# ndrwmlnk/critic-guided-segmentation-of-rewarding-objects-in-first-person-views

Hardware: AMD Instinct MI355X
Metric: Hourglass+critic train images/sec, 64x64x3 batch=512 (higher is better)
Workload: dtype f32

## Files before the change

critic-guided-segmentation-of-rewarding-objects-in-first-person-views_amd/csrc/mask_head.hip:

```cpp
#include "wgrad_body.h"

struct MHeadParams {
    const float* dzpre; const float* h; const float* w2; const float* w0;
    const void* img;
    const float* o0;
    float* dh;
    float* d_o0;
    float* slab2;
    float* slab0;
    int n, ntiles;
    unsigned long long* dbg;
};

#ifdef CGS_DEBUG_STAMPS
#define MH_T() __builtin_amdgcn_s_memtime()
static unsigned long long* g_mh_stamps = nullptr;
extern "C" int dbg_mask_head_stamps(unsigned long long* stamps) { g_mh_stamps = stamps; return CGS_OK; }
#else
#define MH_T() 0ull
#endif

#ifndef MH_WACC_PK
#define MH_WACC_PK 1
#endif
#ifndef MH_APK
#define MH_APK 1
#endif
#ifndef MH_INTERLEAVE
#define MH_INTERLEAVE 1
#endif
#ifndef MH_DGRAD4
#define MH_DGRAD4 1
#endif
#ifndef MH_DZWIN
#define MH_DZWIN 1
#endif
template <int TH, bool W0>
struct MHeadGeo {
    static constexpr int H = 64, W = 64, TRA = TH + 2, PW = W + 2, PS = 17, DZW = W + 4, DZR = TH + 4, STRIPS = H / TH;
    static constexpr int XT = TRA * PW * PS, DZ = DZR * DZW;
    static constexpr int W4P = MH_DGRAD4 ? 16 * 16 * 8 : 24 * 16 * 16;
    static constexpr int LR = TH / 2 + 2, LC = W / 2 + 2;
    static constexpr int XIMG = W0 ? TRA * PW * 4 : 0, XO = W0 ? LR * LC * 8 : 0;
    static constexpr int FLOATS = 2 * XT + 2 * XIMG + 2 * XO + W4P + 2 * DZ;
    static constexpr size_t LDS = (size_t)((FLOATS + 3) / 4) * 16;
    static constexpr int RED2 = 0, REDA = 1024, REDB = REDA + 4 * 32 * 16, RED_END = REDB + 4 * 4 * 32 * 16;
    static_assert(RED_END <= 2 * XT, "reduction buffers fit in the tile storage");
};

struct MHeadLds { float *xt0, *ximg, *xo, *w4p, *dz; };

template <int TH, bool WG, bool W0, int SRC>
__device__ __forceinline__ void mask_head_builder(const MHeadParams& P, const MHeadLds& L, const int btid, const int T,
                                                  const int bid, const int grid) {
    using G = MHeadGeo<TH, W0>;
    constexpr int H = G::H, W = G::W, TRA = G::TRA, PW = G::PW, PS = G::PS, DZW = G::DZW, LR = G::LR, LC = G::LC;
    constexpr int IT = TRA * W * 4 / 256, DIT = (G::DZ + 255) / 256;
    constexpr int NPIX = TRA * PW, NLO = LR * LC * 2, ITA = (NPIX + 255) / 256, ITB = (NLO + 255) / 256;
    static_assert((TRA * W * 4) % 256 == 0, "whole iterations: no element is visited twice");
    const int lane = btid & 63, wave = btid >> 6;
    const int pl = btid & 3;
    static_assert(4 * W == 256, "one tile row per 256-thread item");
    const int bx = btid >> 2, bx4 = btid;
    auto tile_of = [&](int i) { return bid + (i < T ? i : T - 1) * grid; };

    float w2r[9][4];
#if MH_APK
    typedef float mh_f2 __attribute__((ext_vector_type(2)));
    mh_f2 w2p[9][2];
#endif
#if MH_WACC_PK
#if !MH_APK
    typedef float mh_f2 __attribute__((ext_vector_type(2)));
#endif
    mh_f2 wacc[9][2];
#else
    float wacc[9][4];
#endif
    float bacc = 0.f;
    float4 hvs[IT];
    float dzr[DIT];
#pragma unroll
    for (int t = 0; t < 9; ++t)
#pragma unroll
        for (int c = 0; c < 4; ++c) {
            w2r[t][c] = P.w2[t * 16 + 4 * pl + c];
#if MH_APK
            w2p[t][c >> 1][c & 1] = w2r[t][c];
#endif
#if MH_WACC_PK
            wacc[t][c >> 1][c & 1] = 0.f;
#else
            wacc[t][c] = 0.f;
#endif
        }

    auto load_h_into = [&](float4 (&dst)[IT], int tile) {
        const int n0 = tile / G::STRIPS, row0 = (tile % G::STRIPS) * TH;
#pragma unroll
        for (int it = 0; it < IT; ++it) {
            const int y = row0 + it - 1;
            const bool in = y >= 0 && y < H;
            dst[it] = ((const float4*)P.h)[(in ? (n0 * H + y) * W * 4 : 0) + bx4];
        }
    };
    auto load_h = [&](int tile) { load_h_into(hvs, tile); };
    auto load_dz = [&](int tile) {
        const int n0 = tile / G::STRIPS, row0 = (tile % G::STRIPS) * TH;
#pragma unroll
        for (int it = 0; it < DIT; ++it) {
            int e = btid + it * 256;
            e = e < G::DZ ? e : G::DZ - 1;
            int y = row0 + e / DZW - 2, x = e % DZW - 2;
            bool in = y >= 0 && y < H && x >= 0 && x < W;
            dzr[it] = P.dzpre[in ? (n0 * H + y) * W + x : 0];
        }
    };
    auto store_dz = [&](int tile, int buf) {
        const int row0 = (tile % G::STRIPS) * TH;
        float* const dzb = L.dz + buf * G::DZ;
#pragma unroll
        for (int it = 0; it < DIT; ++it) {
            int e = btid + it * 256;
            e = e < G::DZ ? e : G::DZ - 1;
            int y = row0 + e / DZW - 2, x = e % DZW - 2;
            bool in = y >= 0 && y < H && x >= 0 && x < W;
            dzb[e] = in ? dzr[it] : 0.f;
        }
    };

    [[maybe_unused]] float4 ra[W0 ? ITA : 1], rb[W0 ? ITB : 1];
    auto fetch_x = [&](int tile) {
        const int n0 = tile / G::STRIPS, row0 = (tile % G::STRIPS) * TH;
#pragma unroll
        for (int it = 0; it < ITA; ++it) {
            int e = btid + it * 256; e = e < NPIX ? e : NPIX - 1;
            int y = row0 + e / PW - 1, x = e % PW - 1;
            bool in = y >= 0 && y < H && x >= 0 && x < W;
            int pix = in ? (n0 * H + y) * W + x : 0;
            if constexpr (SRC == WSRC_U8) {
                const uint32_t* s32 = (const uint32_t*)P.img;
                int off = pix * 3, last = P.n * H * W * 3 / 4 - 1, d = off >> 2;
                ra[it].x = __uint_as_float(s32[d]);
                ra[it].y = __uint_as_float(s32[d + 1 <= last ? d + 1 : last]);
            } else {
                const float* sf = (const float*)P.img;
                ra[it] = make_float4(sf[pix * 3], sf[pix * 3 + 1], sf[pix * 3 + 2], 0.f);
            }
        }
#pragma unroll
        for (int it = 0; it < ITB; ++it) {
            int e = btid + it * 256; e = e < NLO ? e : NLO - 1;
            int half = e & 1, pc = (e >> 1) % LC, pr = (e >> 1) / LC;
            int ly = row0 / 2 + pr - 1, lx = pc - 1;
            bool in = ly >= 0 && ly < H / 2 && lx >= 0 && lx < W / 2;
            rb[it] = ((const float4*)P.o0)[in ? ((n0 * (H / 2) + ly) * (W / 2) + lx) * 2 + half : 0];
        }
    };
    auto commit_x = [&](int tile, int buf) {
        const int n0 = tile / G::STRIPS, row0 = (tile % G::STRIPS) * TH;
        float4* const ximg4 = (float4*)(L.ximg + buf * G::XIMG);
        float4* const xo4 = (float4*)(L.xo + buf * G::XO);
#pragma unroll
        for (int it = 0; it < ITA; ++it) {
            int e = btid + it * 256; e = e < NPIX ? e : NPIX - 1;
            int y = row0 + e / PW - 1, x = e % PW - 1;
            bool in = y >= 0 && y < H && x >= 0 && x < W;
            float4 v = ra[it];
            if constexpr (SRC == WSRC_U8) {
                int pix = in ? (n0 * H + y) * W + x : 0;
                const uint32_t lo = __float_as_uint(v.x), hi = __float_as_uint(v.y);
                const uint32_t b3 = __builtin_amdgcn_alignbyte(hi, lo, (uint32_t)((pix * 3) & 3));
                const float sc = 1.f / 255.f;
                v = make_float4((float)(b3 & 255u) * sc, (float)((b3 >> 8) & 255u) * sc, (float)((b3 >> 16) & 255u) * sc, 0.f);
            }
            v.w = 0.f;
            ximg4[e] = in ? v : f4zero();
        }
#pragma unroll
        for (int it = 0; it < ITB; ++it) {
            int e = btid + it * 256; e = e < NLO ? e : NLO - 1;
            int pc = (e >> 1) % LC, pr = (e >> 1) / LC;
            int ly = row0 / 2 + pr - 1, lx = pc - 1;
            bool in = ly >= 0 && ly < H / 2 && lx >= 0 && lx < W / 2;
            xo4[e] = in ? rb[it] : f4zero();
        }
    };
    load_dz(tile_of(0));
    load_h(tile_of(0));
    store_dz(tile_of(0), 0);
    __syncthreads();

    [[maybe_unused]] unsigned long long tp = MH_T(), s_p1 = 0, s_w1 = 0, s_p2 = 0, s_w2 = 0;
    for (int i = 0; i <= T; ++i) {
        [[maybe_unused]] const unsigned long long tb = MH_T();
        [[maybe_unused]] unsigned long long tc = tb;
        if (i < T) {
            const int tile = tile_of(i);
            const int n0 = tile / G::STRIPS, row0 = (tile % G::STRIPS) * TH;
            float* xt = L.xt0 + (i & 1) * G::XT;
            const float* dz = L.dz + (i & 1) * G::DZ;
            load_dz(tile_of(i + 1));
            if constexpr (W0) fetch_x(tile);
            __builtin_amdgcn_sched_barrier(0);
#ifdef MH_WHATIF_NOBUILD
            if (P.n < 0)
#endif
            {
#if MH_DZWIN
            float dzw[IT + 2][3];
#pragma unroll
            for (int rr = 0; rr < IT + 2; ++rr)
#pragma unroll
                for (int cc = 0; cc < 3; ++cc) dzw[rr][cc] = dz[rr * DZW + bx + 1 + cc];
            __builtin_amdgcn_sched_barrier(0);
#endif
#pragma unroll
            for (int it = 0; it < IT; ++it) {
                const int r = it;
                const int x = bx, y = row0 + it - 1;
                const bool in = (it >= 1 && it <= TH) || (y >= 0 && y < H);
                const int gi = (in ? (n0 * H + y) * W * 4 : 0) + bx4;
                const float4 hv = hvs[it];
                const bool own = it >= 1 && it <= TH;
                const float4 hw_ = own ? hv : f4zero();
#if MH_APK
                mh_f2 a01 = {0.f, 0.f}, a23 = {0.f, 0.f};
#else
                float a0 = 0.f, a1 = 0.f, a2 = 0.f, a3 = 0.f;
#endif
#pragma unroll
                for (int ky = 0; ky < 3; ++ky)
#pragma unroll
                    for (int kx = 0; kx < 3; ++kx) {
#if MH_DZWIN
                        float d = dzw[r + 2 - ky][2 - kx];
#else
                        float d = dz[(r + 2 - ky) * DZW + x + 3 - kx];
#endif
#if MH_APK
                        {
                            const mh_f2 dd = {d, d};
                            a01 = __builtin_elementwise_fma(dd, w2p[ky * 3 + kx][0], a01);
                            a23 = __builtin_elementwise_fma(dd, w2p[ky * 3 + kx][1], a23);
                        }
#else
                        a0 = fmaf(d, w2r[ky * 3 + kx][0], a0); a1 = fmaf(d, w2r[ky * 3 + kx][1], a1);
                        a2 = fmaf(d, w2r[ky * 3 + kx][2], a2); a3 = fmaf(d, w2r[ky * 3 + kx][3], a3);
#endif
                        if (WG && it != 0 && it != IT - 1) {
#if MH_WACC_PK
                            const mh_f2 dd = {d, d};
                            wacc[ky * 3 + kx][0] = __builtin_elementwise_fma(dd, mh_f2{hw_.x, hw_.y}, wacc[ky * 3 + kx][0]);
                            wacc[ky * 3 + kx][1] = __builtin_elementwise_fma(dd, mh_f2{hw_.z, hw_.w}, wacc[ky * 3 + kx][1]);
#else
                            wacc[ky * 3 + kx][0] = fmaf(d, hw_.x, wacc[ky * 3 + kx][0]);
                            wacc[ky * 3 + kx][1] = fmaf(d, hw_.y, wacc[ky * 3 + kx][1]);
                            wacc[ky * 3 + kx][2] = fmaf(d, hw_.z, wacc[ky * 3 + kx][2]);
                            wacc[ky * 3 + kx][3] = fmaf(d, hw_.w, wacc[ky * 3 + kx][3]);
#endif
                        }
                    }
#if MH_APK
                const float a0 = a01[0], a1 = a01[1], a2 = a23[0], a3 = a23[1];
#endif
                static_assert(IT == TH + 2, "one item per tile row: item index == row index");
                if (WG && it != 0 && it != IT - 1) {
#if MH_DZWIN
                    bacc += (own && pl == 0) ? dzw[r + 1][1] : 0.f;
#else
                    bacc += (own && pl == 0) ? dz[(r + 1) * DZW + x + 2] : 0.f;
#endif
#pragma unroll
                    for (int t = 0; t < 9; ++t)
#pragma unroll
#if MH_WACC_PK
                        for (int c = 0; c < 2; ++c) asm volatile("" : "+v"(wacc[t][c]));
#else
                        for (int c = 0; c < 4; ++c) asm volatile("" : "+v"(wacc[t][c]));
#endif
                }
                float4 v = make_float4(a0 * (hv.x > 0.f ? 1.f : 0.01f), a1 * (hv.y > 0.f ? 1.f : 0.01f),
                                       a2 * (hv.z > 0.f ? 1.f : 0.01f), a3 * (hv.w > 0.f ? 1.f : 0.01f));
                v = in ? v : f4zero();
                float* d = xt + (r * PW + x + 1) * PS + 4 * pl;
                d[0] = v.x; d[1] = v.y; d[2] = v.z; d[3] = v.w;
                if (own && P.dh) ((float4*)P.dh)[gi] = v;
                __builtin_amdgcn_sched_barrier(0);
            }
            }
            load_h(tile_of(i + 1));
            tc = MH_T();
            store_dz(tile_of(i + 1), (i + 1) & 1);
            if constexpr (W0) commit_x(tile, i & 1);
        }
        [[maybe_unused]] const unsigned long long te = MH_T();
        __syncthreads();
        if (CGS_STAMP_PTR(P.dbg)) { const unsigned long long td = MH_T(); s_p1 += te - tc; s_p2 += tc - tb; s_w2 += td - te; tp = td; }
    }
    if (CGS_STAMP_PTR(P.dbg) && btid == 0) {
        unsigned long long* o = CGS_STAMP_PTR(P.dbg) + (size_t)bid * 16;
        o[0] = s_p1; o[1] = s_w1; o[2] = s_p2; o[3] = s_w2; o[4] = (unsigned long long)T;
    }

    if constexpr (WG) {
        float* red2 = L.xt0 + G::RED2;
#pragma unroll
        for (int t = 0; t < 9; ++t)
#pragma unroll
            for (int c = 0; c < 4; ++c) {
#if MH_WACC_PK
                float v = wacc[t][c >> 1][c & 1];
#else
                float v = wacc[t][c];
#endif
                v += __shfl_xor(v, 4, 64); v += __shfl_xor(v, 8, 64); v += __shfl_xor(v, 16, 64); v += __shfl_xor(v, 32, 64);
                if (lane < 4) red2[(wave * 4 + lane) * 37 + t * 4 + c] = v;
            }
        float v = bacc;
        v += __shfl_xor(v, 4, 64); v += __shfl_xor(v, 8, 64); v += __shfl_xor(v, 16, 64); v += __shfl_xor(v, 32, 64);
        if (lane < 4) red2[(wave * 4 + lane) * 37 + 36] = v;
    }
}

template <int TH, bool W0, int SRC>
__device__ __forceinline__ void mask_head_matrix(const MHeadParams& P, const MHeadLds& L, const int mtid, const int T,
                                                 const int bid, const int grid) {
    using G = MHeadGeo<TH, W0>;
    constexpr int PW = G::PW, PS = G::PS, LC = G::LC;
    static_assert(TH == 8, "4 matrix waves: one low-res row (data gradient) and one even + one odd row (weight gradient) each");
    const int lane = mtid & 63, mwave = mtid >> 6;
    const int l15 = lane & 15, kq = lane >> 4;
    auto tile_of = [&](int i) { return bid + (i < T ? i : T - 1) * grid; };
    frag4 accA[2], accB[2][2][2];
#pragma unroll
    for (int q = 0; q < 2; ++q) {
        accA[q] = frag4{0.f, 0.f, 0.f, 0.f};
#pragma unroll
        for (int c = 0; c < 4; ++c) accB[c >> 1][c & 1][q] = frag4{0.f, 0.f, 0.f, 0.f};
    }
    int rimg[2];
#pragma unroll
    for (int q = 0; q < 2; ++q) {
        int r = 16 * q + l15, tap = r / 3, c = r % 3;
        rimg[q] = r < 27 ? ((tap / 3) * PW + tap % 3) * 4 + c : 0;
    }
    const float m1 = (16 + l15 < 27) ? 1.f : 0.f, m0 = (16 + l15 == 27) ? 1.f : 0.f;

    [[maybe_unused]] float w4r[2][16];
    if constexpr (MH_DGRAD4) {
        if (mwave < 2) {
#pragma unroll
            for (int g = 0; g < 2; ++g)
#pragma unroll
                for (int k = 0; k < 16; ++k) w4r[g][k] = L.w4p[(k * 16 + (lane >> 2)) * 8 + 4 * g + (lane & 3)];
        }
    }
    [[maybe_unused]] unsigned long long tp = MH_T(), s_p1 = 0, s_w1 = 0, s_dg = 0, s_wg = 0, s_w2 = 0, tm = 0;
    __syncthreads();
    for (int i = 0; i <= T; ++i) {
        [[maybe_unused]] const unsigned long long ta = MH_T();
        [[maybe_unused]] const unsigned long long tb = ta;
        if (i > 0) {
            const int tile = tile_of(i - 1);
            const int n0 = tile / G::STRIPS, row0 = (tile % G::STRIPS) * TH;
            const float* xt = L.xt0 + ((i - 1) & 1) * G::XT;
            [[maybe_unused]] const float* const ximg = L.ximg + ((i - 1) & 1) * G::XIMG;
            [[maybe_unused]] const float* const xo = L.xo + ((i - 1) & 1) * G::XO;
#ifdef MH_WHATIF_NODGRAD
            if (P.n < 0)
#endif
            if constexpr (MH_DGRAD4) {
                if (mwave < 2) {
                    const int qyl = 2 * mwave + (lane >> 5), qx = lane & 31;
                    const float* bp = xt + ((2 * qyl) * PW + 2 * qx) * PS;
                    frag4 d0 = frag4{0.f, 0.f, 0.f, 0.f}, d1 = frag4{0.f, 0.f, 0.f, 0.f};
                    float bv[2][16];
                    auto ldp = [&](int k, int buf) {
#pragma unroll
                        for (int oc = 0; oc < 16; ++oc) bv[buf][oc] = bp[((k >> 2) * PW + (k & 3)) * PS + oc];
                    };
                    ldp(0, 0);
                    static_for<16>([&](auto K) {
                        constexpr int k = decltype(K)::value;
                        if constexpr (k + 1 < 16) ldp(k + 1, (k + 1) & 1);
                        __builtin_amdgcn_sched_barrier(0);
                        static_for<16>([&](auto OC) {
                            constexpr int oc = decltype(OC)::value;
                            d0 = __builtin_amdgcn_mfma_f32_4x4x1f32(w4r[0][k], bv[k & 1][oc], d0, 4, oc, 0);
                            d1 = __builtin_amdgcn_mfma_f32_4x4x1f32(w4r[1][k], bv[k & 1][oc], d1, 4, oc, 0);
                        });
                        __builtin_amdgcn_sched_barrier(0);
                    });
                    float4* o = (float4*)(P.d_o0 + ((size_t)(n0 * 32 + row0 / 2 + qyl) * 32 + qx) * 8);
                    o[0] = make_float4(d0[0], d0[1], d0[2], d0[3]);
                    o[1] = make_float4(d1[0], d1[1], d1[2], d1[3]);
                }
            } else {
                const int qyl = mwave;
                const int abase = ((2 * qyl) * PW + 4 * l15) * PS + kq;
                const float* wb = L.w4p + kq * 16 + l15;
                frag4 d = frag4{0.f, 0.f, 0.f, 0.f}, d1 = frag4{0.f, 0.f, 0.f, 0.f};
                constexpr int GS = 12, NG = 96 / GS;
                float av[2][GS], bw[2][GS];
                auto ld = [&](int g, int buf) {
#pragma unroll
                    for (int j = 0; j < GS; ++j) {
                        const int s = g * GS + j, pos = s >> 2, u = pos / 6, v6 = pos % 6;
                        av[buf][j] = xt[abase + (u * PW + v6) * PS + 4 * (s & 3)];
                        bw[buf][j] = wb[s * 64];
                    }
                };
                ld(0, 0);
                __builtin_amdgcn_sched_barrier(0);
#pragma unroll
                for (int g = 0; g < NG; ++g) {
                    if (g + 1 < NG) ld(g + 1, (g + 1) & 1);
#if !MH_INTERLEAVE
                    __builtin_amdgcn_sched_barrier(0);
#endif
#pragma unroll
                    for (int j = 0; j < GS; j += 2) {
                        d = __builtin_amdgcn_mfma_f32_16x16x4f32(av[g & 1][j], bw[g & 1][j], d, 0, 0, 0);
                        d1 = __builtin_amdgcn_mfma_f32_16x16x4f32(av[g & 1][j + 1], bw[g & 1][j + 1], d1, 0, 0, 0);
                    }
#if MH_INTERLEAVE
                    if (g + 1 < NG) {
#pragma unroll
                        for (int j = 0; j < GS; ++j) {
                            __builtin_amdgcn_sched_group_barrier(0x008, 1, 0);
                            __builtin_amdgcn_sched_group_barrier(0x100, 1, 0);
                        }
                    } else {
                        __builtin_amdgcn_sched_group_barrier(0x008, GS, 0);
                    }
#endif
                    __builtin_amdgcn_sched_barrier(0);
                }
                d += d1;
                float* o = P.d_o0 + ((size_t)(n0 * 32 + row0 / 2 + qyl) * 32 + 2 * (4 * kq)) * 8 + l15;
#pragma unroll
                for (int j = 0; j < 4; ++j) o[j * 16] = d[j];
            }
            if (CGS_STAMP_PTR(P.dbg)) tm = MH_T();
#ifdef MH_WHATIF_NOWGRAD
            if (P.n < 0)
#endif
            if constexpr (W0) {
                constexpr int UU = 2, CPP = 8 / UU, NCH = 4 * CPP;
                const int bb = (PW + 1 + 2 * kq) * PS + l15;
                const int ib = (2 * kq) * 4;
                const int ob = kq * 8 + l15;
                float ai[2][UU][2], ao[2][UU][2], b[2][UU];
                auto do_half = [&](int rp, auto PY) {
                    constexpr int py = decltype(PY)::value;
                    const int yl = 2 * rp + py;
                    auto ld = [&](int ch, int buf) {
                        const int px = ch / CPP, s0 = UU * (ch % CPP);
#pragma unroll
                        for (int u = 0; u < UU; ++u) b[buf][u] = xt[bb + (yl * PW + px + 8 * (s0 + u)) * PS];
#pragma unroll
                        for (int q = 0; q < 2; ++q)
#pragma unroll
                            for (int u = 0; u < UU; ++u) ai[buf][u][q] = ximg[ib + rimg[q] + (yl * PW + px + 8 * (s0 + u)) * 4];
#pragma unroll
                        for (int q = 0; q < 2; ++q)
#pragma unroll
                            for (int u = 0; u < UU; ++u) ao[buf][u][q] = xo[ob + ((rp + q + py) * LC + px + 4 * (s0 + u)) * 8];
                    };
                    ld(0, 0);
#pragma unroll
                    for (int ch = 0; ch < 2 * CPP; ++ch) {
                        if (ch + 1 < 2 * CPP) ld(ch + 1, (ch + 1) & 1);
                        __builtin_amdgcn_sched_barrier(0);
                        const int px = ch / CPP;
#pragma unroll
                        for (int u = 0; u < UU; ++u) {
                            const float bv = b[ch & 1][u];
                            accA[0] = __builtin_amdgcn_mfma_f32_16x16x4f32(ai[ch & 1][u][0], bv, accA[0], 0, 0, 0);
                            accA[1] = __builtin_amdgcn_mfma_f32_16x16x4f32(fmaf(ai[ch & 1][u][1], m1, m0), bv, accA[1], 0, 0, 0);
                            accB[py][px][0] = __builtin_amdgcn_mfma_f32_16x16x4f32(ao[ch & 1][u][0], bv, accB[py][px][0], 0, 0, 0);
                            accB[py][px][1] = __builtin_amdgcn_mfma_f32_16x16x4f32(ao[ch & 1][u][1], bv, accB[py][px][1], 0, 0, 0);
                        }
                        __builtin_amdgcn_sched_barrier(0);
                    }
                };
                const int h_lo = MH_DGRAD4 ? (mwave < 2 ? mwave : 2 + 3 * (mwave - 2)) : 2 * mwave;
                const int h_n = MH_DGRAD4 ? (mwave < 2 ? 1 : 3) : 2;
#pragma unroll 1
                for (int hh = h_lo; hh < h_lo + h_n; ++hh) {
                    if (hh & 1) do_half(hh >> 1, std::integral_constant<int, 1>{});
                    else do_half(hh >> 1, std::integral_constant<int, 0>{});
                }
            }
        }
        [[maybe_unused]] const unsigned long long tc = MH_T();
        __syncthreads();
        if (CGS_STAMP_PTR(P.dbg)) {
            const unsigned long long td = MH_T();
            s_w2 += td - tc; tp = td;
            if (i > 0) { s_dg += tm - tb; s_wg += tc - tm; } else s_dg += tc - tb;
        }
    }
    if (CGS_STAMP_PTR(P.dbg) && mtid == 0) {
        unsigned long long* o = CGS_STAMP_PTR(P.dbg) + (size_t)bid * 16 + 8;
        o[0] = s_p1; o[1] = s_w1; o[2] = s_dg; o[3] = s_wg; o[4] = s_w2;
    }

    if constexpr (W0) {
        float* redA = L.xt0 + G::REDA + mwave * (32 * 16);
        float* redB = L.xt0 + G::REDB + mwave * (4 * 32 * 16);
#pragma unroll
        for (int q = 0; q < 2; ++q)
#pragma unroll
            for (int j = 0; j < 4; ++j) {
                const int r = 16 * q + 4 * kq + j;
                redA[r * 16 + l15] = accA[q][j];
#pragma unroll
                for (int c = 0; c < 4; ++c) redB[(c * 32 + r) * 16 + l15] = accB[c >> 1][c & 1][q][j];
            }
    }
}

template <int TH, bool WG, bool W0, int SRC>
__global__ void __launch_bounds__(512) mask_head_kernel(MHeadParams P) {
    if (CGS_KARG_PREFETCH) cgs_kernarg_prefetch<sizeof(MHeadParams)>();
    using G = MHeadGeo<TH, W0>;
    constexpr int TRA = G::TRA, PW = G::PW, PS = G::PS;
    extern __shared__ __attribute__((aligned(16))) float4 smem[];
    MHeadLds L;
    L.xt0 = (float*)smem;
    L.ximg = L.xt0 + 2 * G::XT;
    L.xo = L.ximg + 2 * G::XIMG;
    L.w4p = L.xo + 2 * G::XO;
    L.dz = L.w4p + G::W4P;
    const int tid = threadIdx.x;
    [[maybe_unused]] const unsigned long long t_start = MH_T();

    static_assert(G::W4P % 512 == 0 && G::W4P / 512 <= 12, "table rounds");
    {
        float wv[G::W4P / 512][4];
        auto decode = [&](int e, int& u, int& v, int& oc, int& c) {
            if constexpr (MH_DGRAD4) { c = e & 7; oc = (e >> 3) & 15; const int pos = e >> 7; u = pos >> 2; v = pos & 3; }
            else { const int col = e & 15, pos = e >> 8; oc = (e >> 4) & 15; u = pos / 6; c = col & 7; v = pos % 6 - 2 * (col >> 3); }
        };
#pragma unroll
        for (int k = 0; k < G::W4P / 512; ++k) {
            int u, v, oc, c;
            decode(tid + 512 * k, u, v, oc, c);
#pragma unroll
            for (int ab = 0; ab < 4; ++ab) {
                const int ky = (ab >> 1) + 2 - u, kx = (ab & 1) + 2 - v;
                const bool ok = v >= 0 && v <= 3 && ky >= 0 && ky <= 2 && kx >= 0 && kx <= 2;
                wv[k][ab] = P.w0[ok ? ((ky * 3 + kx) * 11 + 3 + c) * 16 + oc : 0];
            }
        }
#pragma unroll
        for (int k = 0; k < G::W4P / 512; ++k) {
            int u, v, oc, c;
            decode(tid + 512 * k, u, v, oc, c);
            float sm = 0.f;
#pragma unroll
            for (int ab = 0; ab < 4; ++ab) {
                const int ky = (ab >> 1) + 2 - u, kx = (ab & 1) + 2 - v;
                const bool ok = v >= 0 && v <= 3 && ky >= 0 && ky <= 2 && kx >= 0 && kx <= 2;
                sm += ok ? wv[k][ab] : 0.f;
            }
            L.w4p[tid + 512 * k] = sm;
        }
    }
    for (int e = tid; e < 2 * TRA * 2 * 16; e += 512) {
        int ch = e & 15, side = (e >> 4) & 1, r = (e >> 5) % TRA, bufi = e / (32 * TRA);
        L.xt0[bufi * G::XT + (r * PW + (side ? PW - 1 : 0)) * PS + ch] = 0.f;
    }
    __syncthreads();

    const int grid = gridDim.x, bid = blockIdx.x;
    const int T = (P.ntiles - bid + grid - 1) / grid;
    if (CGS_STAMP_PTR(P.dbg) && tid == 0) { CGS_STAMP_PTR(P.dbg)[(size_t)bid * 16 + 5] = t_start; CGS_STAMP_PTR(P.dbg)[(size_t)bid * 16 + 6] = MH_T(); }
    if (__builtin_amdgcn_readfirstlane(tid) < 256) mask_head_builder<TH, WG, W0, SRC>(P, L, tid, T, bid, grid);
    else mask_head_matrix<TH, W0, SRC>(P, L, tid - 256, T, bid, grid);
    __syncthreads();
    [[maybe_unused]] const unsigned long long t_after_roles = MH_T();

    if constexpr (W0) {
        const float* redA = L.xt0 + G::REDA;
        const float* redB = L.xt0 + G::REDB;
        auto sum4 = [&](const float* p, int stride) { return (p[0] + p[stride]) + (p[2 * stride] + p[3 * stride]); };
        for (int e = tid; e < 1600; e += 512) {
            float v;
            if (e >= 1584) {
                v = sum4(redA + 27 * 16 + (e - 1584), 32 * 16);
            } else {
                const int oc = e & 15, ci = (e >> 4) % 11, tap = (e >> 4) / 11, ky = tap / 3, kx = tap % 3;
                if (ci < 3) {
                    v = sum4(redA + (tap * 3 + ci) * 16 + oc, 32 * 16);
                } else {
                    v = 0.f;
#pragma unroll
                    for (int c = 0; c < 4; ++c) {
                        const int py = c >> 1, px = c & 1;
                        const int a = py == 0 ? (ky >= 1) : (ky == 2), b = px == 0 ? (kx >= 1) : (kx == 2);
                        v += sum4(redB + (c * 32 + (a * 2 + b) * 8 + (ci - 3)) * 16 + oc, 4 * 32 * 16);
                    }
                }
            }
            P.slab0[(size_t)blockIdx.x * 1600 + e] = v;
        }
    }
    if constexpr (WG) {
        const float* red2 = L.xt0 + G::RED2;
        if (tid < 145) {
            int t = tid / 16, ch = tid % 16, p = ch >> 2, c = ch & 3;
            int idx = (tid < 144) ? t * 4 + c : 36;
            if (tid == 144) p = 0;
            float v = (red2[(0 * 4 + p) * 37 + idx] + red2[(1 * 4 + p) * 37 + idx]) + (red2[(2 * 4 + p) * 37 + idx] + red2[(3 * 4 + p) * 37 + idx]);
            P.slab2[(size_t)blockIdx.x * 145 + tid] = v;
        }
    }
    if (CGS_STAMP_PTR(P.dbg) && tid == 0) { CGS_STAMP_PTR(P.dbg)[(size_t)blockIdx.x * 16 + 7] = MH_T(); CGS_STAMP_PTR(P.dbg)[(size_t)blockIdx.x * 16 + 13] = t_after_roles; }
}

static int mask_head_blocks(int n) { int t = n * (64 / 8); return t < 256 ? t : 256; }
int mask_head_slabs(int n) { return n <= 0 ? 0 : mask_head_blocks(n); }

template <bool WG, bool W0, int SRC>
static int launch_mask_head(MHeadParams P, hipStream_t st) {
    constexpr int TH = 8;
    using G = MHeadGeo<TH, W0>;
    P.ntiles = P.n * G::STRIPS;
    static hipError_t attr = hipFuncSetAttribute(reinterpret_cast<const void*>(&mask_head_kernel<TH, WG, W0, SRC>),
                                                 hipFuncAttributeMaxDynamicSharedMemorySize, (int)G::LDS);
    if (attr != hipSuccess) return (int)attr;
    hipLaunchKernelGGL((mask_head_kernel<TH, WG, W0, SRC>), dim3(mask_head_blocks(P.n)), dim3(512), G::LDS, st, P);
    CGS_HIP_CHECK_LAUNCH();
    return CGS_OK;
}

int mask_head_launch(int n, int img_kind, const void* img, const float* o0, const float* dzpre, const float* h,
                     const float* w2, const float* w0, float* dh, float* d_o0, float* slab2, float* slab0, hipStream_t st) {
    if (n <= 0) return CGS_OK;
    MHeadParams P{dzpre, h, w2, w0, img, o0, dh, d_o0, slab2, slab0, n, 0, nullptr};
#ifdef CGS_DEBUG_STAMPS
    P.dbg = g_mh_stamps;
#endif
    if (slab0) {
        if (!slab2 || !img || !o0) return CGS_ERR_BADARG;
        return img_kind == CGS_SRC_U8 ? launch_mask_head<true, true, WSRC_U8>(P, st) : launch_mask_head<true, true, WSRC_F32>(P, st);
    }
    return slab2 ? launch_mask_head<true, false, WSRC_F32>(P, st) : launch_mask_head<false, false, WSRC_F32>(P, st);
}
```

Before: 1.004 million.

## Assign contiguous row strips per block and carry halo rows between tiles

Each block now gets a contiguous run of tiles instead of a grid-strided set, so consecutive tiles are usually vertically adjacent strips of the same image. The builder carries the last two computed h/dh rows and the dz halo rows into the next tile instead of reloading and recomputing them. The last halo row's weight-gradient contribution is accumulated directly, and the x fetch is moved to a fixed point inside the build loop so its loads overlap compute. This cuts redundant global loads and halo recompute, at the cost of more branching and register pressure, plus possible load imbalance from the contiguous assignment.

```diff
diff --git a/critic-guided-segmentation-of-rewarding-objects-in-first-person-views_amd/csrc/mask_head.hip b/critic-guided-segmentation-of-rewarding-objects-in-first-person-views_amd/csrc/mask_head.hip
--- a/critic-guided-segmentation-of-rewarding-objects-in-first-person-views_amd/csrc/mask_head.hip
+++ b/critic-guided-segmentation-of-rewarding-objects-in-first-person-views_amd/csrc/mask_head.hip
@@ -19,6 +19,9 @@
 #else
 #define MH_T() 0ull
 #endif
+#ifndef MH_STAMP_WAVE
+#define MH_STAMP_WAVE 0
+#endif
 
 #ifndef MH_WACC_PK
 #define MH_WACC_PK 1
@@ -35,6 +38,16 @@
 #ifndef MH_DZWIN
 #define MH_DZWIN 1
 #endif
+#ifndef MH_ROWS
+#define MH_ROWS 1
+#endif
+#ifndef MH_FETCH_AT
+#define MH_FETCH_AT 3
+#endif
+#ifndef MH_ROWS_DZ
+#define MH_ROWS_DZ 1
+#endif
+static_assert(MH_ROWS || !MH_ROWS_DZ, "MH_ROWS_DZ needs MH_ROWS");
 template <int TH, bool W0>
 struct MHeadGeo {
     static constexpr int H = 64, W = 64, TRA = TH + 2, PW = W + 2, PS = 17, DZW = W + 4, DZR = TH + 4, STRIPS = H / TH;
@@ -52,7 +65,7 @@
 
 template <int TH, bool WG, bool W0, int SRC>
 __device__ __forceinline__ void mask_head_builder(const MHeadParams& P, const MHeadLds& L, const int btid, const int T,
-                                                  const int bid, const int grid) {
+                                                  const int bid, const int t0, const int tstep) {
     using G = MHeadGeo<TH, W0>;
     constexpr int H = G::H, W = G::W, TRA = G::TRA, PW = G::PW, PS = G::PS, DZW = G::DZW, LR = G::LR, LC = G::LC;
     constexpr int IT = TRA * W * 4 / 256, DIT = (G::DZ + 255) / 256;
@@ -62,7 +75,7 @@
     const int pl = btid & 3;
     static_assert(4 * W == 256, "one tile row per 256-thread item");
     const int bx = btid >> 2, bx4 = btid;
-    auto tile_of = [&](int i) { return bid + (i < T ? i : T - 1) * grid; };
+    auto tile_of = [&](int i) { return t0 + (i < T ? i : T - 1) * tstep; };
 
     float w2r[9][4];
 #if MH_APK
@@ -95,34 +108,45 @@
 #endif
         }
 
-    auto load_h_into = [&](float4 (&dst)[IT], int tile) {
+    auto load_h_into = [&](float4 (&dst)[IT], int tile, const bool carried) {
         const int n0 = tile / G::STRIPS, row0 = (tile % G::STRIPS) * TH;
 #pragma unroll
         for (int it = 0; it < IT; ++it) {
+            if (MH_ROWS && it < 2 && carried) continue;
             const int y = row0 + it - 1;
             const bool in = y >= 0 && y < H;
             dst[it] = ((const float4*)P.h)[(in ? (n0 * H + y) * W * 4 : 0) + bx4];
         }
     };
-    auto load_h = [&](int tile) { load_h_into(hvs, tile); };
-    auto load_dz = [&](int tile) {
+    auto load_h = [&](int tile, const bool carried) { load_h_into(hvs, tile, carried); };
+    static_assert(!MH_ROWS_DZ || (G::DZ - 2 * DZW <= (DIT - 1) * 256 && 2 * DZW <= 256), "dz tile items");
+    auto dz_elem = [&](int it) {
+        if (MH_ROWS_DZ) {
+            if (it == DIT - 1) return btid < 2 * DZW ? btid : 2 * DZW - 1;
+            const int e = 2 * DZW + btid + it * 256;
+            return e < G::DZ ? e : G::DZ - 1;
+        }
+        const int e = btid + it * 256;
+        return e < G::DZ ? e : G::DZ - 1;
+    };
+    auto load_dz = [&](int tile, const bool carried) {
         const int n0 = tile / G::STRIPS, row0 = (tile % G::STRIPS) * TH;
 #pragma unroll
         for (int it = 0; it < DIT; ++it) {
-            int e = btid + it * 256;
-            e = e < G::DZ ? e : G::DZ - 1;
+            if (MH_ROWS_DZ && it == DIT - 1 && carried) continue;
+            const int e = dz_elem(it);
             int y = row0 + e / DZW - 2, x = e % DZW - 2;
             bool in = y >= 0 && y < H && x >= 0 && x < W;
             dzr[it] = P.dzpre[in ? (n0 * H + y) * W + x : 0];
         }
     };
-    auto store_dz = [&](int tile, int buf) {
+    auto store_dz = [&](int tile, int buf, const bool carried) {
         const int row0 = (tile % G::STRIPS) * TH;
         float* const dzb = L.dz + buf * G::DZ;
 #pragma unroll
         for (int it = 0; it < DIT; ++it) {
-            int e = btid + it * 256;
-            e = e < G::DZ ? e : G::DZ - 1;
+            if (MH_ROWS_DZ && it == DIT - 1 && carried) continue;
+            const int e = dz_elem(it);
             int y = row0 + e / DZW - 2, x = e % DZW - 2;
             bool in = y >= 0 && y < H && x >= 0 && x < W;
             dzb[e] = in ? dzr[it] : 0.f;
@@ -186,9 +210,9 @@
             xo4[e] = in ? rb[it] : f4zero();
         }
     };
-    load_dz(tile_of(0));
-    load_h(tile_of(0));
-    store_dz(tile_of(0), 0);
+    load_dz(tile_of(0), false);
+    load_h(tile_of(0), false);
+    store_dz(tile_of(0), 0, false);
     __syncthreads();
 
     [[maybe_unused]] unsigned long long tp = MH_T(), s_p1 = 0, s_w1 = 0, s_p2 = 0, s_w2 = 0;
@@ -200,8 +224,10 @@
             const int n0 = tile / G::STRIPS, row0 = (tile % G::STRIPS) * TH;
             float* xt = L.xt0 + (i & 1) * G::XT;
             const float* dz = L.dz + (i & 1) * G::DZ;
-            load_dz(tile_of(i + 1));
-            if constexpr (W0) fetch_x(tile);
+            const bool c_in = MH_ROWS && i > 0 && row0 != 0;
+            const bool c_out = MH_ROWS && i + 1 < T && row0 != H - TH;
+            load_dz(tile_of(i + 1), c_out);
+            if constexpr (W0 && !MH_ROWS) fetch_x(tile);
             __builtin_amdgcn_sched_barrier(0);
 #ifdef MH_WHATIF_NOBUILD
             if (P.n < 0)
@@ -209,14 +235,21 @@
             {
 #if MH_DZWIN
             float dzw[IT + 2][3];
-#pragma unroll
-            for (int rr = 0; rr < IT + 2; ++rr)
+            if (!c_in) {
+#pragma unroll
+                for (int rr = 0; rr < 2; ++rr)
+#pragma unroll
+                    for (int cc = 0; cc < 3; ++cc) dzw[rr][cc] = dz[rr * DZW + bx + 1 + cc];
+            }
+#pragma unroll
+            for (int rr = 2; rr < IT + 2; ++rr)
 #pragma unroll
                 for (int cc = 0; cc < 3; ++cc) dzw[rr][cc] = dz[rr * DZW + bx + 1 + cc];
             __builtin_amdgcn_sched_barrier(0);
 #endif
-#pragma unroll
-            for (int it = 0; it < IT; ++it) {
+            auto dh_row = [&](int r) { return xt + (r * PW + bx + 1) * PS + 4 * pl; };
+            auto build_item = [&](auto IT_) {
+                constexpr int it = decltype(IT_)::value;
                 const int r = it;
                 const int x = bx, y = row0 + it - 1;
                 const bool in = (it >= 1 && it <= TH) || (y >= 0 && y < H);
@@ -265,11 +298,29 @@
                 const float a0 = a01[0], a1 = a01[1], a2 = a23[0], a3 = a23[1];
 #endif
                 static_assert(IT == TH + 2, "one item per tile row: item index == row index");
-                if (WG && it != 0 && it != IT - 1) {
+                if (WG && ((it != 0 && it != IT - 1) || (MH_ROWS && it == IT - 1 && c_out))) {
+                    if (it == IT - 1) {
+#pragma unroll
+                        for (int t = 0; t < 9; ++t) {
 #if MH_DZWIN
-                    bacc += (own && pl == 0) ? dzw[r + 1][1] : 0.f;
-#else
-                    bacc += (own && pl == 0) ? dz[(r + 1) * DZW + x + 2] : 0.f;
+                            const float d = dzw[r + 2 - t / 3][2 - t % 3];
+#else
+                            const float d = dz[(r + 2 - t / 3) * DZW + x + 3 - t % 3];
+#endif
+#if MH_WACC_PK
+                            const mh_f2 dd = {d, d};
+                            wacc[t][0] = __builtin_elementwise_fma(dd, mh_f2{hv.x, hv.y}, wacc[t][0]);
+                            wacc[t][1] = __builtin_elementwise_fma(dd, mh_f2{hv.z, hv.w}, wacc[t][1]);
+#else
+                            wacc[t][0] = fmaf(d, hv.x, wacc[t][0]); wacc[t][1] = fmaf(d, hv.y, wacc[t][1]);
+                            wacc[t][2] = fmaf(d, hv.z, wacc[t][2]); wacc[t][3] = fmaf(d, hv.w, wacc[t][3]);
+#endif
+                        }
+                    }
+#if MH_DZWIN
+                    bacc += ((own || it == IT - 1) && pl == 0) ? dzw[r + 1][1] : 0.f;
+#else
+                    bacc += ((own || it == IT - 1) && pl == 0) ? dz[(r + 1) * DZW + x + 2] : 0.f;
 #endif
 #pragma unroll
                     for (int t = 0; t < 9; ++t)
@@ -283,22 +334,39 @@
                 float4 v = make_float4(a0 * (hv.x > 0.f ? 1.f : 0.01f), a1 * (hv.y > 0.f ? 1.f : 0.01f),
                                        a2 * (hv.z > 0.f ? 1.f : 0.01f), a3 * (hv.w > 0.f ? 1.f : 0.01f));
                 v = in ? v : f4zero();
-                float* d = xt + (r * PW + x + 1) * PS + 4 * pl;
+                if constexpr (MH_ROWS && it >= IT - 2) hvs[it - (IT - 2)] = v;
+                float* d = dh_row(r);
                 d[0] = v.x; d[1] = v.y; d[2] = v.z; d[3] = v.w;
-                if (own && P.dh) ((float4*)P.dh)[gi] = v;
+                if ((own || (MH_ROWS && it == IT - 1 && c_out)) && P.dh) ((float4*)P.dh)[gi] = v;
                 __builtin_amdgcn_sched_barrier(0);
-            }
-            }
-            load_h(tile_of(i + 1));
+            };
+            if (c_in) {
+#pragma unroll
+                for (int r = 0; r < 2; ++r) {
+                    float* d = dh_row(r);
+                    d[0] = hvs[r].x; d[1] = hvs[r].y; d[2] = hvs[r].z; d[3] = hvs[r].w;
+                }
+                __builtin_amdgcn_sched_barrier(0);
+            } else {
+                build_item(std::integral_constant<int, 0>{});
+                build_item(std::integral_constant<int, 1>{});
+            }
+            static_for<IT - 2>([&](auto K) {
+                constexpr int it = decltype(K)::value + 2;
+                build_item(std::integral_constant<int, it>{});
+                if constexpr (W0 && MH_ROWS && it == MH_FETCH_AT) { fetch_x(tile); __builtin_amdgcn_sched_barrier(0); }
+            });
+            }
+            load_h(tile_of(i + 1), c_out);
             tc = MH_T();
-            store_dz(tile_of(i + 1), (i + 1) & 1);
+            store_dz(tile_of(i + 1), (i + 1) & 1, c_out);
             if constexpr (W0) commit_x(tile, i & 1);
         }
         [[maybe_unused]] const unsigned long long te = MH_T();
         __syncthreads();
         if (CGS_STAMP_PTR(P.dbg)) { const unsigned long long td = MH_T(); s_p1 += te - tc; s_p2 += tc - tb; s_w2 += td - te; tp = td; }
     }
-    if (CGS_STAMP_PTR(P.dbg) && btid == 0) {
+    if (CGS_STAMP_PTR(P.dbg) && btid == 64 * MH_STAMP_WAVE) {
         unsigned long long* o = CGS_STAMP_PTR(P.dbg) + (size_t)bid * 16;
         o[0] = s_p1; o[1] = s_w1; o[2] = s_p2; o[3] = s_w2; o[4] = (unsigned long long)T;
     }
@@ -325,13 +393,13 @@
 
 template <int TH, bool W0, int SRC>
 __device__ __forceinline__ void mask_head_matrix(const MHeadParams& P, const MHeadLds& L, const int mtid, const int T,
-                                                 const int bid, const int grid) {
+                                                 const int bid, const int t0, const int tstep) {
     using G = MHeadGeo<TH, W0>;
     constexpr int PW = G::PW, PS = G::PS, LC = G::LC;
     static_assert(TH == 8, "4 matrix waves: one low-res row (data gradient) and one even + one odd row (weight gradient) each");
     const int lane = mtid & 63, mwave = mtid >> 6;
     const int l15 = lane & 15, kq = lane >> 4;
-    auto tile_of = [&](int i) { return bid + (i < T ? i : T - 1) * grid; };
+    auto tile_of = [&](int i) { return t0 + (i < T ? i : T - 1) * tstep; };
     frag4 accA[2], accB[2][2][2];
 #pragma unroll
     for (int q = 0; q < 2; ++q) {
@@ -502,7 +570,7 @@
             if (i > 0) { s_dg += tm - tb; s_wg += tc - tm; } else s_dg += tc - tb;
         }
     }
-    if (CGS_STAMP_PTR(P.dbg) && mtid == 0) {
+    if (CGS_STAMP_PTR(P.dbg) && mtid == 64 * MH_STAMP_WAVE) {
         unsigned long long* o = CGS_STAMP_PTR(P.dbg) + (size_t)bid * 16 + 8;
         o[0] = s_p1; o[1] = s_w1; o[2] = s_dg; o[3] = s_wg; o[4] = s_w2;
     }
@@ -576,10 +644,15 @@
     __syncthreads();
 
     const int grid = gridDim.x, bid = blockIdx.x;
-    const int T = (P.ntiles - bid + grid - 1) / grid;
+#if MH_ROWS
+    const int tq = P.ntiles / grid, tr = P.ntiles - tq * grid;
+    const int T = tq + (bid < tr ? 1 : 0), t0 = bid * tq + (bid < tr ? bid : tr), tstep = 1;
+#else
+    const int T = (P.ntiles - bid + grid - 1) / grid, t0 = bid, tstep = grid;
+#endif
     if (CGS_STAMP_PTR(P.dbg) && tid == 0) { CGS_STAMP_PTR(P.dbg)[(size_t)bid * 16 + 5] = t_start; CGS_STAMP_PTR(P.dbg)[(size_t)bid * 16 + 6] = MH_T(); }
-    if (__builtin_amdgcn_readfirstlane(tid) < 256) mask_head_builder<TH, WG, W0, SRC>(P, L, tid, T, bid, grid);
-    else mask_head_matrix<TH, W0, SRC>(P, L, tid - 256, T, bid, grid);
+    if (__builtin_amdgcn_readfirstlane(tid) < 256) mask_head_builder<TH, WG, W0, SRC>(P, L, tid, T, bid, t0, tstep);
+    else mask_head_matrix<TH, W0, SRC>(P, L, tid - 256, T, bid, t0, tstep);
     __syncthreads();
     [[maybe_unused]] const unsigned long long t_after_roles = MH_T();
 
```

Result: no change. 1.003 million (median of 2 runs) (-0.0%).
